# roclark/torchsr

Hardware: AMD Instinct MI355X
Metric: 96x96 HR crops/sec (SRGAN GAN train step) (higher is better)
Workload: dtype f32; 1 GPU; SRGAN full GAN step (Generator + Discriminator + VGG19 perceptual loss), 96x96 HR crops, batch 16 per GPU, fp32; per_gpu_batch=16, global_batch=16, crop=96, parallelism=dp1, hip_graph=True, vgg19_weights=seeded-random, plan_cus=256

## Files before the change

include/srx.h:

```cpp
#ifndef SRX_H
#define SRX_H

#include <stddef.h>
#include <stdint.h>

#ifdef __cplusplus
extern "C" {
#endif

#define SRX_VERSION 100

enum {
  SRX_OK = 0,
  SRX_E_BADARG = 1,
  SRX_E_UNSUPPORTED = 2,
  SRX_E_HIP = 3,
  SRX_E_WORKSPACE = 4
};

enum { SRX_ACT_NONE = 0, SRX_ACT_RELU = 1, SRX_ACT_LRELU = 2, SRX_ACT_PRELU = 3 };

int srx_version(void);
int srx_last_error(char* buf, size_t n);
int srx_build_info(char* buf, size_t n);
// ... 35 lines not shown
} srx_conv2d_t;

size_t srx_conv2d_packed_fwd_floats(const srx_conv2d_t* d);
size_t srx_conv2d_packed_bwd_floats(const srx_conv2d_t* d);
size_t srx_conv2d_fwd_ws_floats(const srx_conv2d_t* d);
size_t srx_conv2d_bwd_data_ws_floats(const srx_conv2d_t* d);
size_t srx_conv2d_bwd_weight_ws_floats(const srx_conv2d_t* d);
int srx_conv2d_stat_rows(const srx_conv2d_t* d);

int srx_conv2d_plan(const srx_conv2d_t* d, int which, int* out);

int srx_conv2d_force_plan(int bm, int bn, int split, int ks);
int srx_conv2d_force_s2(int mode, int bm, int bn);
int srx_wgrad_force(int lin, int nsplit);
int srx_wgrad_force_kernels(int dma, int rows, int reduce);
int srx_thin_force_rows(int rows);
int srx_linear_force(int form, int splits);

int srx_thin_plan(const srx_conv2d_t* d, int which, int* out);

int srx_linear_plan(int B, int K, int J, int which, int* out);

int srx_wgrad_plan(const srx_conv2d_t* d, int nprob, int per_out, int* out);

int srx_conv2d_pack(const srx_conv2d_t* d, const float* w_oihw, float* wpk_fwd, float* wpk_bwd, void* stream);

size_t srx_pack_table_bytes(int n_layers);
int srx_pack_table_build(const srx_conv2d_t* descs, int n, const float* const* w_oihw, float* const* wpk_fwd,
                         float* const* wpk_bwd, void* host_table, int* n_records, long long* max_elems);
int srx_pack_table_run(const void* dev_table, int n_records, long long max_elems, void* stream);
// ... 277 lines not shown
```

torchsr_amd/_lib.py:

```python
import ctypes as C
import os
import subprocess
import sys

_HERE = os.path.dirname(os.path.abspath(__file__))
CSRC = os.path.join(_HERE, 'csrc')
LIB_PATH = os.environ.get('SRX_LIB') or os.path.join(CSRC, 'libsrx_hip.so')
SOURCES = ['api.cpp', 'gconv.hip', 'wgrad.hip', 'convpack.hip', 'c64.hip', 'thin9.hip', 'rdb.hip', 'thin.hip', 'rowtile.hip', 'augment.hip', 'degrade.hip', 'norm.hip', 'eltwise.hip', 'linear.hip', 'loss.hip', 'head.hip', 'wino.hip', 'optim.hip', 'dihedral.hip', 'resample.hip', 'usm.hip', 'pool.hip', 'colorfix.hip', 'compact.hip', 'specnorm.hip']
HEADERS = ['srx_common.h', 'conv_host.h', os.path.join('..', '..', 'include', 'srx.h')]

ACT_NONE, ACT_RELU, ACT_LRELU, ACT_PRELU = 0, 1, 2, 3


class Conv2dDesc(C.Structure):
    _fields_ = [
        ('N', C.c_int32), ('H', C.c_int32), ('W', C.c_int32),
        ('Cin', C.c_int32), ('Cin_s', C.c_int32), ('Cout', C.c_int32), ('Cout_s', C.c_int32),
        ('KH', C.c_int32), ('KW', C.c_int32), ('stride', C.c_int32), ('pad', C.c_int32),
        ('shuffle', C.c_int32), ('act', C.c_int32), ('slope', C.c_float), ('up', C.c_int32),
        ('precision', C.c_int32),
    ]


class DgradEpilogue(C.Structure):
# ... 120 lines not shown
    'srx_plane_moments': (_I, [_P, _L, _I, _I, _P, _Z, _P, _P]),
    'srx_color_fix_adain_apply': (_I, [_P, _P, _L, _I, _I, _P, _P, _P]),
    'srx_conv2d_packed_fwd_floats': (_Z, [_D]),
    'srx_conv2d_packed_bwd_floats': (_Z, [_D]),
    'srx_conv2d_fwd_ws_floats': (_Z, [_D]),
    'srx_conv2d_bwd_data_ws_floats': (_Z, [_D]),
    'srx_conv2d_bwd_weight_ws_floats': (_Z, [_D]),
    'srx_conv2d_stat_rows': (_I, [_D]),
    'srx_conv2d_plan': (_I, [_D, _I, C.POINTER(C.c_int)]),
    'srx_conv2d_force_plan': (_I, [_I, _I, _I, _I]),
    'srx_thin_plan': (_I, [_D, _I, C.POINTER(C.c_int)]),
    'srx_thin_force_rows': (_I, [_I]),
    'srx_conv2d_force_s2': (_I, [_I, _I, _I]),
    'srx_wgrad_force': (_I, [_I, _I]),
    'srx_wgrad_force_kernels': (_I, [_I, _I, _I]),
    'srx_wgrad_plan': (_I, [_D, _I, _I, C.POINTER(C.c_int)]),
    'srx_linear_force': (_I, [_I, _I]),
    'srx_linear_plan': (_I, [_I, _I, _I, _I, C.POINTER(C.c_int)]),
    'srx_pack_table_bytes': (_Z, [_I]),
    'srx_pack_table_build': (_I, [_P, _I, _P, _P, _P, _P, C.POINTER(C.c_int), C.POINTER(C.c_longlong)]),
    'srx_pack_table_add_wino': (_I, [_P, C.POINTER(C.c_int), C.POINTER(C.c_longlong), _D, _P, _P, _I]),
    'srx_pack_table_run': (_I, [_P, _I, C.c_longlong, _P]),
    'srx_conv2d_pack': (_I, [_D, _P, _P, _P, _P]),
    'srx_conv2d_fwd': (_I, [_D, _P, _P, _P, _P, _P, _P, _Z, _P]),
    'srx_conv3x3_c64_bf16_packed_bytes': (_Z, [_I]),
    'srx_conv3x3_c64_bf16_pack': (_I, [_P, _P, _P, _I, _I, _P, _P]),
    'srx_conv3x3_c64_bf16_fwd': (_I, [_I, _I, _I, _I, _I, _P, _P, _F, _P, _P, _I, _P]),
    'srx_conv3x3_c64_bf16_plan': (_I, [_I, _I, _I, _I, C.POINTER(C.c_int)]),
    'srx_f32_to_bf16': (_I, [_P, _P, _L, _P]),
    'srx_bf16_to_f32': (_I, [_P, _P, _L, _P]),
# ... 200 lines not shown
```

torchsr_amd/csrc/api.cpp:

```cpp
#include "srx_common.h"
#include <cstdarg>
#include <cstdio>
#include <atomic>
#include <cstdlib>
#include <cstring>
#include <mutex>
#include <vector>

static thread_local char g_err[512] = "";

void srx_set_error(const char* fmt, ...) {
  va_list ap;
  va_start(ap, fmt);
  vsnprintf(g_err, sizeof(g_err), fmt, ap);
  va_end(ap);
}

extern "C" int srx_version(void) { return SRX_VERSION; }

#ifndef SRX_SOURCES_SHA256
#define SRX_SOURCES_SHA256 "unknown"
#endif
static const char g_build_info[] = "srx-build-sources-sha256:" SRX_SOURCES_SHA256;
extern "C" int srx_build_info(char* buf, size_t n) {
// ... 3 lines not shown
  return SRX_OK;
}

static SrxDevSwitches read_switches() {
  SrxDevSwitches s{};
  auto flag = [](const char* n) { const char* e = getenv(n); return e != nullptr && e[0] != 0 && !(e[0] == '0' && e[1] == 0); };
  auto num = [](const char* n) { const char* e = getenv(n); return e ? atoi(e) : 0; };
  s.no_rt36 = flag("SRX_NO_RT36");
  s.no_wgrad_rows = flag("SRX_NO_WGRAD_ROWS");
  s.no_bn_bwd_fuse = flag("SRX_NO_BN_BWD_FUSE");
  s.no_bn_fwd_fuse = flag("SRX_NO_BN_FWD_FUSE");
  s.no_first3 = flag("SRX_NO_FIRST3");
  s.no_c64 = flag("SRX_NO_C64");
  s.no_wgrad_dma = flag("SRX_NO_WGRAD_DMA");
  s.no_wgrad_lin = flag("SRX_NO_WGRAD_LIN");
  s.wgrad_nsplit = num("SRX_WGRAD_NSPLIT");
  s.wgrad_rows_nsplit = num("SRX_WGRAD_ROWS_NSPLIT");
  s.first3_wgs_per_cu = num("SRX_FIRST3_WGS_PER_CU");
  s.thin_fwd_rows = num("SRX_THIN_FWD_ROWS");
  s.reserved_cus = num("SRX_RESERVED_CUS");
  s.c64_ablate = num("SRX_C64_ABLATE");
  s.rdb_ablate = num("SRX_RDB_ABLATE");
  s.no_wino = flag("SRX_NO_WINO");
  s.old_wgrad_reduce = flag("SRX_OLD_WGRAD_REDUCE");
  s.wino_no_tail = flag("SRX_WINO_NO_TAIL");
  s.wino_zsplit = num("SRX_WINO_ZSPLIT");
  s.wino_bn = num("SRX_WINO_BN");
  s.s2_mode = num("SRX_S2_MODE");
  if (s.rdb_ablate != 0 || s.c64_ablate != 0) {
    const char* ok = getenv("SRX_ALLOW_GARBAGE_RESULTS");
// ... 142 lines not shown
```

torchsr_amd/csrc/conv_host.h:

```cpp
#pragma once
#include "srx_common.h"
#include <atomic>

constexpr int BK = 32;

struct Geo {
  int Ho, Wo, Ck, K, Kp, Cnp, cps;
};

struct BwdClass {
  int ph, pw, nth, ntw, dminh, dminw, Hm, Wm, K, Kp;
  size_t woff;
};

int check_desc(const srx_conv2d_t* d);
bool small_enough(const srx_conv2d_t* d);
int pad_rows(int c);
Geo fwd_geo(const srx_conv2d_t* d);
int bwd_ck(const srx_conv2d_t* d);
int bwd_classes(const srx_conv2d_t* d, BwdClass* cls, size_t& total_floats);
srx_conv2d_t upsampled_desc(const srx_conv2d_t* d);
size_t upsampled_floats(const srx_conv2d_t* d);

struct ConvForce {
  std::atomic<int> plan[4];
  std::atomic<int> s2[3];
  std::atomic<int> wg[2];
  std::atomic<int> wg_rows;
  std::atomic<int> wk[3];
};
ConvForce& conv_force();
```

torchsr_amd/csrc/gconv.hip:

```cpp
#include "conv_host.h"
#include <cstdio>
#include <cstdlib>
#include <algorithm>
#include <mutex>
#include <type_traits>
#include <utility>
#include <vector>

namespace {

struct GArgs {
  const float* in; const float* w; const float* bias; float* out; float* part;
  int N, Hi, Wi, Ci;
  int Hm, Wm, M, HmWm;
  float inv_HmWm, inv_Wm;
  int in_stride, nth, ntw, dh0, dw0, Ck, K, Kp;
  int Cn, Cs;
  int Ho, Wo, Co;
  int out_stride, oh_off, ow_off;
  int out_shuffle, in_shuffle;
  int up;
  int act; float slope;
  int linear_out;
  int mtiles;
// ... 1067 lines not shown
  srx_conv2d_t h = *d;
  h.up = 0; h.H = 2 * d->H; h.W = 2 * d->W;
  return h;
}
size_t upsampled_floats(const srx_conv2d_t* d) { return (size_t)d->N * 2 * d->H * 2 * d->W * d->Cin_s; }

ConvForce& conv_force() {
  static ConvForce* f = [] {
    ConvForce* s = new ConvForce;
    const SrxDevSwitches& e = srx_dev();
    for (int i = 0; i < 4; ++i) s->plan[i].store(e.force_plan ? e.plan[i] : 0);
    s->s2[0].store((e.s2_mode & 1) ? 1 : 0); s->s2[1].store(0); s->s2[2].store(0);
    s->wg[0].store(e.no_wgrad_lin ? 0 : -1); s->wg[1].store(e.wgrad_nsplit > 0 && e.wgrad_nsplit <= 64 ? e.wgrad_nsplit : 0);
    s->wg_rows.store(e.wgrad_rows_nsplit > 0 && e.wgrad_rows_nsplit <= 64 ? e.wgrad_rows_nsplit : 0);
    s->wk[0].store(e.no_wgrad_dma ? 0 : -1); s->wk[1].store(e.no_wgrad_rows ? 0 : -1); s->wk[2].store(e.old_wgrad_reduce ? 0 : -1);
    return s;
  }();
  return *f;
}

namespace {

struct Plan { int BM, BN, mtiles, ntiles, tiles, full, tail, split, kc_per_split, ks; float cost; bool refused; };

enum Family { F_GCONV, F_BIG, F_MULTI, F_S2F, NFAM };
constexpr unsigned char K1 = 1, K2 = 2, K4 = 4, K12 = K1 | K2;
struct Tile {
  int BM, BN, WM, WN, XR;
  float eff;
  unsigned char ks[NFAM][4];
// ... 489 lines not shown

extern "C" int srx_conv2d_force_s2(int mode, int bm, int bn) {
  SRX_REQUIRE(((mode == 0 || mode == 1) && bm == 0 && bn == 0) ||
              (mode == 2 && ((bm == 0 && bn == 0) || tile_sides_known(F_S2F, bm, bn))),
              "conv2d_force_s2: (0, 0, 0), (1, 0, 0) or (2, BM 64 / 128 / 144, BN 64 / 128) -- (2, 0, 0): the model's fused tile");
  ConvForce& f = conv_force();
  f.s2[0].store(0);
  f.s2[1].store(bm); f.s2[2].store(bn); f.s2[0].store(mode);
  return SRX_OK;
}

extern "C" int srx_wgrad_force(int lin, int nsplit) {
  SRX_REQUIRE(lin >= -1 && lin <= 1 && nsplit >= 0 && nsplit <= 64, "wgrad_force: LIN -1 / 0 / 1, 0..64 row splits");
  ConvForce& f = conv_force();
  f.wg[0].store(lin); f.wg[1].store(nsplit); f.wg_rows.store(nsplit);
  return SRX_OK;
}

extern "C" int srx_wgrad_force_kernels(int dma, int rows, int reduce) {
  SRX_REQUIRE(dma >= -1 && dma <= 1 && rows >= -1 && rows <= 1 && reduce >= -1 && reduce <= 1,
              "wgrad_force_kernels: DMA staging, image-row kernel, row-wise reduction: each -1 / 0 / 1");
  ConvForce& f = conv_force();
  f.wk[0].store(dma); f.wk[1].store(rows); f.wk[2].store(reduce);
  return SRX_OK;
}

static int conv_fwd_impl(const srx_conv2d_t* d, const float* x, const float* wpk, const float* bias, const float* residual,
                         float out_scale, float* y, float* bn_partials, float* ws, size_t ws_floats, void* stream) {
  if (int rc = check_desc(d)) return rc;
  SRX_REQUIRE(x && wpk && y, "conv2d_fwd: null pointer");
// ... 360 lines not shown
```

torchsr_amd/csrc/srx_common.h:

```cpp
#pragma once
#include <hip/hip_runtime.h>
#include <hip/hip_ext.h>
#include <stdint.h>
#include <stddef.h>
#include "../../include/srx.h"

typedef float f32x4 __attribute__((ext_vector_type(4)));
typedef float f32x16 __attribute__((ext_vector_type(16)));

void srx_set_error(const char* fmt, ...);

#define SRX_FAIL(code, ...)      \
  do {                           \
    srx_set_error(__VA_ARGS__);  \
    return (code);               \
  } while (0)

#define SRX_REQUIRE(cond, ...) \
  do {                         \
    if (!(cond)) SRX_FAIL(SRX_E_BADARG, __VA_ARGS__); \
  } while (0)

#define SRX_CHECK_LAUNCH(name)                                                        \
  do {                                                                                \
    hipError_t e__ = hipGetLastError();                                               \
    if (e__ != hipSuccess) SRX_FAIL(SRX_E_HIP, "%s: %s", name, hipGetErrorString(e__)); \
  } while (0)

struct SrxDevSwitches {
  bool no_rt36, no_wgrad_rows, no_bn_bwd_fuse, no_bn_fwd_fuse, no_first3, no_c64, force_plan, no_wgrad_dma, no_wgrad_lin, no_wino, old_wgrad_reduce, wino_no_tail;
  int wgrad_nsplit, wgrad_rows_nsplit, first3_wgs_per_cu, thin_fwd_rows, reserved_cus, c64_ablate, rdb_ablate, wino_zsplit, wino_bn;
  int s2_mode;
  int plan[4];
};
const SrxDevSwitches& srx_dev();
extern "C" int srx_plan_cus(void);

bool srx_prof_on();
bool srx_prof_aux();
bool srx_prof_take(const char* name, double flops, hipEvent_t* e0, hipEvent_t* e1);
#define SRX_LAUNCH_PROF(name, flops, kernel, grid, block, lds, st, ...)                              \
  do {                                                                                               \
    hipEvent_t e0__ = nullptr, e1__ = nullptr;                                                       \
    if (srx_prof_on() && srx_prof_take(name, flops, &e0__, &e1__))                                   \
      hipExtLaunchKernelGGL(kernel, grid, block, (std::uint32_t)(lds), st, e0__, e1__, 0, __VA_ARGS__); \
// ... 91 lines not shown
```

torchsr_amd/csrc/wgrad.hip:

```cpp
#include "conv_host.h"
#include <cstdio>

namespace {

struct WArgs {
  const float* in; const float* dy; float* slab;
  int N, Hi, Wi, Ci, Hm, Wm, M, HmWm;
  float inv_HmWm, inv_Wm;
  int in_stride, nth, ntw, dh0, dw0, Ck, K, Kw;
  int Cd, Cdv, dy_shuffle, Cnw;
  int rows_per_split, ktiles;
  unsigned in_bytes, dy_bytes;
  int s_c, s_rm, dX0, dX1, dX2, dD0, dD1;
  float* bslab;
  int nsplit, nprob;
};

constexpr int WG_MAXP = 72;
struct WMulti {
  WArgs a;
  const float* x[WG_MAXP];
  const float* dy[WG_MAXP];
};
struct WReduce {
// ... 178 lines not shown
  }
  if (want_bias) {
    f32x4* red = reinterpret_cast<f32x4*>(&sD[0][0]);
    red[r0 * 16 + q] = bsum;
    __syncthreads();
    if (tid < 16) {
      f32x4 t = red[tid];
#pragma unroll
      for (int r = 1; r < 16; ++r) t += red[r * 16 + tid];
      *reinterpret_cast<f32x4*>(a.bslab + slab_id * a.Cnw + n0 + 4 * tid) = t;
    }
  }
}

constexpr int WG_MASKW = 768;
template <bool WIDE, bool LIN = false>
__global__ __launch_bounds__(256) void wgrad_dma_kernel(const WMulti mp) {
  static_assert(!LIN || WIDE, "LIN is a form of WIDE");
  const WArgs& a = mp.a;
  typedef unsigned u32x4 __attribute__((ext_vector_type(4)));
  int wi;
  {
    const int W = (int)gridDim.x, b = (int)blockIdx.x, xcd = b & 7, slot = b >> 3, q = W >> 3, r = W & 7;
    wi = (xcd < r ? xcd * (q + 1) : r * (q + 1) + (xcd - r) * q) + slot;
  }
  const int tiles_ = a.ktiles * (a.Cnw / 64);
  const int tile_id = wi % tiles_, rest_ = wi / tiles_;
  const int prob = srx_uniform(rest_ % a.nprob), zsplit = srx_uniform(rest_ / a.nprob);
  constexpr int NSLOT = 3, CHUNK = 32 * 64;
  __shared__ __attribute__((aligned(16))) float sD[NSLOT][CHUNK];
  __shared__ __attribute__((aligned(16))) float sX[NSLOT][CHUNK];
  const int tid = threadIdx.x, lane = tid & 63, wave = srx_uniform(tid >> 6);
  const int ntile = srx_uniform(tile_id / a.ktiles), kt = srx_uniform(tile_id - ntile * a.ktiles);
  const int k0 = kt * 64, n0 = ntile * 64;
  constexpr int NP = WIDE ? 1 : 2;
  const int q = WIDE ? (tid & 7) : (tid & 15), r0 = WIDE ? (tid >> 3) : (tid >> 4);
  auto make_rsrc = [](const void* p, unsigned bytes) {
    const unsigned long long v = (unsigned long long)p;
    u32x4 r;
    r[0] = (unsigned)srx_uniform((int)(unsigned)v);
    r[1] = (unsigned)srx_uniform((int)((unsigned)(v >> 32) & 0xffffu));
    r[2] = bytes;
    r[3] = 0x00020000u;
    return r;
  };
  const u32x4 rx_ = make_rsrc(mp.x[prob], a.in_bytes), rd_ = make_rsrc(mp.dy[prob], a.dy_bytes);

  const int k = k0 + 4 * q;
  const bool kvalid = k < a.K, kvalid1 = WIDE && k + 32 < a.K;
  int dh = 0, dw = 0, kc = 0;
  if (kvalid) {
    const int tap = k / a.Ck;
    kc = k - tap * a.Ck;
    const int th = tap / a.ntw, tw = tap - th * a.ntw;
    dh = a.dh0 + th;
    dw = a.dw0 + tw;
  }
  const int col = n0 + 4 * q;
  const bool cvalid = col < a.Cdv, cvalid1 = WIDE && col + 32 < a.Cdv;
  int sh_i = 0, sh_j = 0, sh_c = col;
  if (a.dy_shuffle) {
    const int ij = col / a.dy_shuffle;
    sh_c = col - ij * a.dy_shuffle;
    sh_i = ij >> 1;
    sh_j = ij & 1;
  }
  const int mbeg = zsplit * a.rows_per_split;
  const int mend = min(a.M, mbeg + a.rows_per_split);

  __shared__ unsigned okmask[LIN ? WG_MASKW : 1];
  if constexpr (LIN) {
    const int nrows = (((mend - mbeg + 31) / 32 + 3) * 32 + 63) & ~63;
    for (int base = wave * 64; base < nrows; base += 256) {
      const int m = mbeg + base + lane;
      int n, rem, mh, mw;
      srx_divmod(m, a.HmWm, a.inv_HmWm, n, rem);
      srx_divmod(rem, a.Wm, a.inv_Wm, mh, mw);
      const bool ok = m < mend && ((unsigned)(mh + dh) < (unsigned)a.Hi) && ((unsigned)(mw + dw) < (unsigned)a.Wi);
      const unsigned long long bits = __ballot(ok);
      if (lane == 0) { okmask[base >> 5] = (unsigned)bits; okmask[(base >> 5) + 1] = (unsigned)(bits >> 32); }
// ... 8 lines not shown
    int n, rem, mh, mw;
    srx_divmod(m, a.HmWm, a.inv_HmWm, n, rem);
    srx_divmod(rem, a.Wm, a.inv_Wm, mh, mw);
    rm[p] = m; rmh[p] = mh; rmw[p] = mw;
    rox[p] = (unsigned)(((n * a.Hi + mh * a.in_stride + dh) * a.Wi + mw * a.in_stride + dw) * a.Ci + kc);
    rod[p] = (unsigned)(a.dy_shuffle ? ((n * 2 * a.Hm + 2 * mh + sh_i) * (2 * a.Wm) + 2 * mw + sh_j) * a.Cd + sh_c
                                     : m * a.Cd + col);
  }
  const unsigned ldsX = (unsigned)(size_t)&sX[0][0], ldsD = (unsigned)(size_t)&sD[0][0];
  auto dma = [&](const u32x4& rs, unsigned voff, unsigned dst) {
    unsigned keep;
    asm volatile("s_mov_b32 %0, m0\n\ts_mov_b32 m0, %2\n\ts_nop 0\n\tbuffer_load_dwordx4 %1, %3, 0 offen lds\n\ts_mov_b32 m0, %0"
                 : "=&s"(keep) : "v"(voff), "s"(dst), "s"(rs) : "memory");
  };
  constexpr unsigned OORL = 0xfffff000u;
  unsigned lin_x = 0, lin_d = 0, lin_w = 0;
  int lin_c = 0;
  if constexpr (LIN) {
    lin_x = 4u * (unsigned)((mbeg + r0 + dh * a.Wi + dw) * a.Ci + kc);
    lin_d = 4u * (unsigned)((mbeg + r0) * a.Cd + col);
    lin_w = okmask[0];
  }
  const unsigned lin_sx = 128u * (unsigned)a.Ci, lin_sd = 128u * (unsigned)a.Cd;
  auto request = [&](int slot) {
    if constexpr (LIN) {
      const bool okx = (lin_w >> r0) & 1u;
      const bool okd = rm[0] < mend;
      const unsigned vx = okx ? lin_x : OORL, vd = okd ? lin_d : OORL;
      const unsigned dst = (unsigned)srx_uniform((int)((unsigned)(slot * CHUNK * 4) + (unsigned)(wave * 1024)));
      dma(rx_, vx, ldsX + dst);
      dma(rd_, vd, ldsD + dst);
      dma(rx_, vx + 128u, ldsX + dst + 4096u);
      dma(rd_, vd + 128u, ldsD + dst + 4096u);
      rm[0] += 32; lin_x += lin_sx; lin_d += lin_sd;
      lin_c += 1;
      lin_w = okmask[lin_c];
      return;
    }
#pragma unroll
    for (int p = 0; p < NP; ++p) {
      const bool valid = rm[p] < mend;
      const int ih = rmh[p] * a.in_stride + dh, iw = rmw[p] * a.in_stride + dw;
      const bool okx = valid && kvalid && ((unsigned)ih < (unsigned)a.Hi) && ((unsigned)iw < (unsigned)a.Wi);
      const unsigned dst = (unsigned)srx_uniform((int)((unsigned)(slot * CHUNK * 4) + (unsigned)(p * 4096 + wave * 1024)));
      dma(rx_, okx ? 4u * rox[p] : 0xffffffffu, ldsX + dst);
      dma(rd_, (valid && cvalid) ? 4u * rod[p] : 0xffffffffu, ldsD + dst);
      if constexpr (WIDE) {
        dma(rx_, (okx && kvalid1) ? 4u * rox[p] + 128u : 0xffffffffu, ldsX + dst + 4096u);
        dma(rd_, (valid && cvalid1) ? 4u * rod[p] + 128u : 0xffffffffu, ldsD + dst + 4096u);
      }
      rm[p] += 32; rmw[p] += a.s_c; rmh[p] += a.s_rm; rox[p] += (unsigned)a.dX0; rod[p] += (unsigned)a.dD0;
      const bool wc = rmw[p] >= a.Wm;
      rmw[p] -= wc ? a.Wm : 0; rmh[p] += wc ? 1 : 0;
      rox[p] += wc ? (unsigned)a.dX1 : 0u; rod[p] += wc ? (unsigned)a.dD1 : 0u;
      const bool wr = rmh[p] >= a.Hm;
      rmh[p] -= wr ? a.Hm : 0;
      rox[p] += wr ? (unsigned)a.dX2 : 0u;
    }
  };
  const bool want_bias = a.bslab != nullptr && kt == 0;
  f32x4 bsum = {0.f, 0.f, 0.f, 0.f}, bsum1 = {0.f, 0.f, 0.f, 0.f};
  f32x16 acc;
#pragma unroll
  for (int r = 0; r < 16; ++r) acc[r] = 0.f;
  const int h = lane >> 5, l31 = lane & 31;
  const int wn = wave >> 1, wk = wave & 1;
  constexpr int SSTEP = WIDE ? 64 : 128, HSTEP = WIDE ? 32 : 64, WSTEP = WIDE ? 1024 : 32;
  auto compute = [&](int slot) {
    const float* cD = &sD[0][0] + slot * CHUNK + h * HSTEP + wn * WSTEP + l31;
    const float* cX = &sX[0][0] + slot * CHUNK + h * HSTEP + wk * WSTEP + l31;
    if (want_bias) {
      if constexpr (WIDE) {
        const float* bd = &sD[0][0] + slot * CHUNK + r0 * 32 + q * 4;
        bsum += *reinterpret_cast<const f32x4*>(bd);
        bsum1 += *reinterpret_cast<const f32x4*>(bd + 1024);
      } else {
        const float* bd = &sD[0][0] + slot * CHUNK + r0 * 64 + q * 4;
        bsum += *reinterpret_cast<const f32x4*>(bd) + *reinterpret_cast<const f32x4*>(bd + 16 * 64);
      }
    }
    float dv[16], xv[16];
#pragma unroll
    for (int s = 0; s < 16; ++s) { dv[s] = cD[s * SSTEP]; xv[s] = cX[s * SSTEP]; }
#pragma unroll
    for (int s = 0; s < 16; ++s) acc = __builtin_amdgcn_mfma_f32_32x32x2f32(dv[s], xv[s], acc, 0, 0, 0);
    __builtin_amdgcn_sched_group_barrier(0x100, 4, 0);
#pragma unroll
    for (int i = 0; i < 8; ++i) {
      __builtin_amdgcn_sched_group_barrier(0x008, 2, 0);
      if (i < 6) __builtin_amdgcn_sched_group_barrier(0x100, 2, 0);
    }
  };
  const int nchunks = (mend - mbeg + 31) / 32;
  request(0);
  request(1);
  asm volatile("s_waitcnt vmcnt(4)" ::: "memory");
  asm volatile("s_waitcnt lgkmcnt(0)\n\ts_barrier" ::: "memory");
  int slot = 0;
  for (int c = 0; c < nchunks; ++c) {
    int s2 = slot + 2; s2 = s2 >= NSLOT ? s2 - NSLOT : s2;
    request(s2);
    compute(slot);
    asm volatile("s_waitcnt vmcnt(4)" ::: "memory");
    asm volatile("s_waitcnt lgkmcnt(0)\n\ts_barrier" ::: "memory");
    slot = slot + 1 == NSLOT ? 0 : slot + 1;
  }
  asm volatile("s_waitcnt vmcnt(0)" ::: "memory");
  const size_t slab_id = (size_t)prob * a.nsplit + zsplit;
  float* slab = a.slab + slab_id * a.Cnw * a.Kw;
#pragma unroll
  for (int r = 0; r < 16; ++r) {
    const int row = n0 + wn * 32 + (r & 3) + 8 * (r >> 2) + 4 * h;
    slab[(size_t)row * a.Kw + k0 + wk * 32 + l31] = acc[r];
  }
  if (want_bias) {
    __syncthreads();
    f32x4* red = reinterpret_cast<f32x4*>(&sD[0][0]);
    constexpr int NR = WIDE ? 32 : 16;
    if constexpr (WIDE) { red[r0 * 16 + q] = bsum; red[r0 * 16 + 8 + q] = bsum1; }
    else red[r0 * 16 + q] = bsum;
    __syncthreads();
    if (tid < 16) {
      f32x4 t = red[tid];
#pragma unroll
      for (int r = 1; r < NR; ++r) t += red[r * 16 + tid];
      *reinterpret_cast<f32x4*>(a.bslab + slab_id * a.Cnw + n0 + 4 * tid) = t;
    }
  }
}

template <int WPX>
__global__ __launch_bounds__(256) void wgrad_rows_bf16_kernel(const WMulti mp) {
  const WArgs& a = mp.a;
  typedef __bf16 bf16x4 __attribute__((ext_vector_type(4)));
  typedef __bf16 bf16x8 __attribute__((ext_vector_type(8)));
  typedef short s16x4 __attribute__((ext_vector_type(4)));
  typedef short s16x8 __attribute__((ext_vector_type(8)));
  typedef s16x4 __attribute__((address_space(3))) * lds_s16x4;
  constexpr int XPS = 64, XROW = (WPX + 2) * XPS;
  constexpr int DPS = 192, DROW = WPX * DPS;
// ... 250 lines not shown
    if (e < nE) {
      const int ci = e / T, tap = e - ci * T;
      const float v = rsum[tap * Ck + ci];
      orow[e] = accumulate ? oldv[i] + v : v;
    }
  }
  for (int e = tid + 256 * PRE; e < nE; e += 256) {
    const int ci = e / T, tap = e - ci * T;
    const float v = rsum[tap * Ck + ci];
    orow[e] = accumulate ? orow[e] + v : v;
  }
}

}

static int wgrad_nsplit(int M, int64_t tiles, int nprob, int Cnw, int Kw, int precision) {
  const int cus = srx_plan_cus();
  const int max_by_rows = (int)srx_cdiv(M, 128);
  int nsplit = 1;
  float best_cost = 1e30f;
  for (int ns = 1; ns <= 64 && ns <= max_by_rows; ++ns) {
    const int rps = (int)srx_roundup(srx_cdiv(M, ns), 32);
    if ((int)srx_cdiv(M, rps) != ns) continue;
    float cost;
    if (precision == 0) {
      const int w = (int)srx_cdiv(tiles * nprob * ns, cus), f = w / 3, r = w - 3 * f;
      cost = (rps / 32 + 3.5f) * (f * 1.696f + (r == 1 ? 0.633f : r == 2 ? 1.177f : 0.f)) + (float)nprob * ns * Cnw * Kw * 8.0f / 50.0e6f;
    } else {
      const int L = (int)srx_cdiv(tiles * nprob * ns, cus);
      const float hide = L >= 4 ? 0.65f : (L == 3 ? 0.7f : (L == 2 ? 0.8f : 1.0f));
      cost = 1.07f * L * (rps / 32 + 6) * hide + (float)nprob * ns * Cnw * Kw * 8.0f / 3.0e6f;
    }
    if (cost < best_cost) { best_cost = cost; nsplit = ns; }
  }
  if (const int v = conv_force().wg[1].load(std::memory_order_relaxed); v > 0) {
    const int rps = (int)srx_roundup(srx_cdiv(M, v), 32);
    if (v > max_by_rows || (int)srx_cdiv(M, rps) != v) {
      srx_set_error("conv2d_bwd_weight: forced %d row splits refused: %d rows split into whole 32-row chunks of at least 128 rows "
                    "give %d splits", v, M, v > max_by_rows ? max_by_rows : (int)srx_cdiv(M, rps));
      return -1;
    }
    nsplit = v;
  }
  const int rps = (int)srx_roundup(srx_cdiv(M, nsplit), 32);
  return (int)srx_cdiv(M, rps);
}

static bool wgrad_rows_ok(const srx_conv2d_t* d) {
  if (conv_force().wk[1].load(std::memory_order_relaxed) == 0 || !d->precision || d->KH != 3 || d->KW != 3 || d->stride != 1 || d->pad != 1 || d->shuffle || d->up == 2) return false;
  return d->Cout == 64 && srx_roundup(d->Cin, 4) % 32 == 0 && (d->W == 32 || d->W == 16);
}
static int wgrad_rows_nsplit(const srx_conv2d_t* d, int nprob) {
  const int cus = srx_plan_cus();
  const int groups = (int)srx_roundup(d->Cin, 4) / 32, rows = d->N * d->H;
  int best = 1;
  float best_cost = 1e30f;
  for (int ns = 1; ns <= 32 && ns <= rows; ++ns) {
    const int rps = (int)srx_cdiv(rows, ns);
// ... 10 lines not shown
    }
    best = v;
  }
  const int rps = (int)srx_cdiv(rows, best);
  return (int)srx_cdiv(rows, rps);
}

enum { WK_F32 = 0, WK_DMA = 1, WK_DMA_WIDE = 2, WK_DMA_LIN = 3, WK_BF16 = 4, WK_ROWS32 = 5, WK_ROWS16 = 6, WK_THIN = 7 };
struct WgradPlan {
  int kernel;
  int nsplit;
  int rows_per_split;
  int reduce;
  int workgroups;
  int Cnw, Kw;
};
static int wgrad_plan(const srx_conv2d_t* d, int nprob, WgradPlan& p) {
  const Geo g = fwd_geo(d);
  const ConvForce& f = conv_force();
  p.Cnw = (int)srx_roundup(d->Cout, 64);
  p.Kw = (int)srx_roundup(g.K, 64);
  const int M = d->N * g.Ho * g.Wo;
  const int64_t tiles = (int64_t)(p.Kw / 64) * (p.Cnw / 64);
  if (wgrad_rows_ok(d)) {
    p.nsplit = wgrad_rows_nsplit(d, nprob);
    if (p.nsplit < 0) return SRX_E_UNSUPPORTED;
    p.kernel = d->W == 32 ? WK_ROWS32 : WK_ROWS16;
    p.rows_per_split = (int)srx_cdiv(d->N * d->H, p.nsplit) * d->W;
    p.workgroups = (g.Ck / 32) * nprob * p.nsplit;
  } else {
    p.nsplit = wgrad_nsplit(M, tiles, nprob, p.Cnw, p.Kw, d->precision);
    if (p.nsplit < 0) return SRX_E_UNSUPPORTED;
    p.rows_per_split = (int)srx_roundup(srx_cdiv(M, p.nsplit), 32);
    p.workgroups = (int)(tiles * nprob * p.nsplit);
    if (d->precision) {
      p.kernel = WK_BF16;
    } else if (f.wk[0].load(std::memory_order_relaxed) == 0) {
      p.kernel = WK_F32;
    } else {
      p.kernel = WK_DMA;
      const int Cdv = bwd_ck(d);
      if (g.Ck % 64 == 0 && Cdv % 64 == 0 && (!g.cps || g.cps % 64 == 0)) {
        const size_t in_bytes = (size_t)d->N * d->H * d->W * d->Cin_s * sizeof(float);
        const size_t dy_bytes = (size_t)M * (d->shuffle ? 4 : 1) * d->Cout_s * sizeof(float);
        const bool lin = f.wg[0].load(std::memory_order_relaxed) != 0 && d->stride == 1 && d->H == g.Ho && d->W == g.Wo && !g.cps &&
                         g.K % 64 == 0 && p.rows_per_split / 32 + 3 <= WG_MASKW && in_bytes < 0xfff00000ull && dy_bytes < 0xfff00000ull;
        p.kernel = lin ? WK_DMA_LIN : WK_DMA_WIDE;
      }
    }
  }
  p.reduce = (f.wk[2].load(std::memory_order_relaxed) == 0 || (size_t)g.K * sizeof(float) > 48 * 1024) ? 0 : 1;
  return SRX_OK;
}

extern "C" int srx_wgrad_plan(const srx_conv2d_t* d, int nprob, int per_out, int* out) {
  if (int rc = check_desc(d)) return rc;
  SRX_REQUIRE(out && nprob >= 1 && nprob <= WG_MAXP && per_out >= 1 && nprob % per_out == 0,
// ... 125 lines not shown
  const double wfl = 2.0 * a.M * d->Cout * a.K * nprob;
  char nm[112];
  if (rows_kernel) {
    if (srx_prof_on()) snprintf(nm, sizeof(nm), "wgrad_rows_bf16_kernel<%d> MxNxK=%dx%dx%d x%d", d->W, a.M, d->Cout, a.K, nprob);
    if (plan.kernel == WK_ROWS32) SRX_LAUNCH_PROF(nm, wfl, wgrad_rows_bf16_kernel<32>, grid, dim3(256), 0, st, mp);
    else SRX_LAUNCH_PROF(nm, wfl, wgrad_rows_bf16_kernel<16>, grid, dim3(256), 0, st, mp);
    SRX_CHECK_LAUNCH("wgrad_rows_bf16_kernel");
  } else {
    const int form = plan.kernel;
    if (srx_prof_on()) {
      if (form == WK_F32 || form == WK_BF16) snprintf(nm, sizeof(nm), "wgrad_kernel<%d> MxNxK=%dx%dx%d x%d", form == WK_BF16 ? 1 : 0, a.M, d->Cout, a.K, nprob);
      else snprintf(nm, sizeof(nm), "wgrad_dma_kernel<%d, %d> MxNxK=%dx%dx%d x%d", form >= WK_DMA_WIDE ? 1 : 0, form == WK_DMA_LIN ? 1 : 0, a.M, d->Cout, a.K, nprob);
    }
    if (form == WK_BF16) SRX_LAUNCH_PROF(nm, wfl, wgrad_kernel<1>, grid, dim3(256), 0, st, mp);
    else if (form == WK_F32) SRX_LAUNCH_PROF(nm, wfl, wgrad_kernel<0>, grid, dim3(256), 0, st, mp);
    else if (form == WK_DMA_LIN) SRX_LAUNCH_PROF(nm, wfl, (wgrad_dma_kernel<true, true>), grid, dim3(256), 0, st, mp);
    else if (form == WK_DMA_WIDE) SRX_LAUNCH_PROF(nm, wfl, wgrad_dma_kernel<true>, grid, dim3(256), 0, st, mp);
    else SRX_LAUNCH_PROF(nm, wfl, wgrad_dma_kernel<false>, grid, dim3(256), 0, st, mp);
    SRX_CHECK_LAUNCH("wgrad_kernel");
  }
  if (plan.reduce == 0) {
    const int64_t n = (int64_t)d->Cout * g.K;
    SRX_LAUNCH_PROF_AUX("wgrad_reduce_kernel", wgrad_reduce_kernel, dim3((unsigned)srx_cdiv(n, 256), (unsigned)nout), dim3(256), 0, st, ws,
                    nsplit * per_out, a.Cnw, a.Kw, g.K, g.Ck, d->Cout, d->Cin, d->KH, d->KW, g.cps, outs, accumulate,
                    a.bslab);
  } else {
    SRX_LAUNCH_PROF_AUX("wgrad_reduce_rows_kernel", wgrad_reduce_rows_kernel, dim3((unsigned)d->Cout, (unsigned)nout), dim3(256),
                    (size_t)g.K * sizeof(float), st, ws, nsplit * per_out, a.Cnw, a.Kw, g.K, g.Ck, d->Cout, d->Cin, d->KH, d->KW, g.cps,
                    outs, accumulate, a.bslab);
  }
// ... 37 lines not shown
```

Measured before the change: 2444 crops/s.

## Add 128x64 tall tile variant to fp32 DMA wgrad kernel with cost-model selection

Adds a TALL template form of the fp32 DMA weight-gradient kernel. Each workgroup computes 128 output channels by 64 K columns, with two MFMA accumulators sharing the same input operand loads. This halves X-tile reloads and workgroup count per output tile. A cost model extension picks the tall tile for eligible 3x3 layers when its estimated cost beats the standard tile by a margin. The trade is more LDS and registers per workgroup, which lowers occupancy, and the selection relies on new empirical constants.

```diff
diff --git a/include/srx.h b/include/srx.h
--- a/include/srx.h
+++ b/include/srx.h
@@ -73,6 +73,7 @@
 int srx_conv2d_force_s2(int mode, int bm, int bn);
 int srx_wgrad_force(int lin, int nsplit);
 int srx_wgrad_force_kernels(int dma, int rows, int reduce);
+int srx_wgrad_force_tile(int tall);
 int srx_thin_force_rows(int rows);
 int srx_linear_force(int form, int splits);
 
diff --git a/torchsr_amd/_lib.py b/torchsr_amd/_lib.py
--- a/torchsr_amd/_lib.py
+++ b/torchsr_amd/_lib.py
@@ -158,6 +158,7 @@
     'srx_conv2d_force_s2': (_I, [_I, _I, _I]),
     'srx_wgrad_force': (_I, [_I, _I]),
     'srx_wgrad_force_kernels': (_I, [_I, _I, _I]),
+    'srx_wgrad_force_tile': (_I, [_I]),
     'srx_wgrad_plan': (_I, [_D, _I, _I, C.POINTER(C.c_int)]),
     'srx_linear_force': (_I, [_I, _I]),
     'srx_linear_plan': (_I, [_I, _I, _I, _I, C.POINTER(C.c_int)]),
diff --git a/torchsr_amd/csrc/api.cpp b/torchsr_amd/csrc/api.cpp
--- a/torchsr_amd/csrc/api.cpp
+++ b/torchsr_amd/csrc/api.cpp
@@ -41,6 +41,7 @@
   s.no_c64 = flag("SRX_NO_C64");
   s.no_wgrad_dma = flag("SRX_NO_WGRAD_DMA");
   s.no_wgrad_lin = flag("SRX_NO_WGRAD_LIN");
+  s.no_wgrad_tall = flag("SRX_NO_WGRAD_TALL");
   s.wgrad_nsplit = num("SRX_WGRAD_NSPLIT");
   s.wgrad_rows_nsplit = num("SRX_WGRAD_ROWS_NSPLIT");
   s.first3_wgs_per_cu = num("SRX_FIRST3_WGS_PER_CU");
diff --git a/torchsr_amd/csrc/conv_host.h b/torchsr_amd/csrc/conv_host.h
--- a/torchsr_amd/csrc/conv_host.h
+++ b/torchsr_amd/csrc/conv_host.h
@@ -28,5 +28,6 @@
   std::atomic<int> wg[2];
   std::atomic<int> wg_rows;
   std::atomic<int> wk[3];
+  std::atomic<int> wg_tile;
 };
 ConvForce& conv_force();
diff --git a/torchsr_amd/csrc/gconv.hip b/torchsr_amd/csrc/gconv.hip
--- a/torchsr_amd/csrc/gconv.hip
+++ b/torchsr_amd/csrc/gconv.hip
@@ -1105,6 +1105,7 @@
     s->wg[0].store(e.no_wgrad_lin ? 0 : -1); s->wg[1].store(e.wgrad_nsplit > 0 && e.wgrad_nsplit <= 64 ? e.wgrad_nsplit : 0);
     s->wg_rows.store(e.wgrad_rows_nsplit > 0 && e.wgrad_rows_nsplit <= 64 ? e.wgrad_rows_nsplit : 0);
     s->wk[0].store(e.no_wgrad_dma ? 0 : -1); s->wk[1].store(e.no_wgrad_rows ? 0 : -1); s->wk[2].store(e.old_wgrad_reduce ? 0 : -1);
+    s->wg_tile.store(e.no_wgrad_tall ? 0 : -1);
     return s;
   }();
   return *f;
@@ -1624,6 +1625,12 @@
   SRX_REQUIRE(lin >= -1 && lin <= 1 && nsplit >= 0 && nsplit <= 64, "wgrad_force: LIN -1 / 0 / 1, 0..64 row splits");
   ConvForce& f = conv_force();
   f.wg[0].store(lin); f.wg[1].store(nsplit); f.wg_rows.store(nsplit);
+  return SRX_OK;
+}
+
+extern "C" int srx_wgrad_force_tile(int tall) {
+  SRX_REQUIRE(tall >= -1 && tall <= 1, "wgrad_force_tile: the 128 x 64 tile -1 (the cost model) / 0 (never) / 1 (wherever eligible)");
+  conv_force().wg_tile.store(tall);
   return SRX_OK;
 }
 
diff --git a/torchsr_amd/csrc/srx_common.h b/torchsr_amd/csrc/srx_common.h
--- a/torchsr_amd/csrc/srx_common.h
+++ b/torchsr_amd/csrc/srx_common.h
@@ -28,7 +28,7 @@
   } while (0)
 
 struct SrxDevSwitches {
-  bool no_rt36, no_wgrad_rows, no_bn_bwd_fuse, no_bn_fwd_fuse, no_first3, no_c64, force_plan, no_wgrad_dma, no_wgrad_lin, no_wino, old_wgrad_reduce, wino_no_tail;
+  bool no_rt36, no_wgrad_rows, no_bn_bwd_fuse, no_bn_fwd_fuse, no_first3, no_c64, force_plan, no_wgrad_dma, no_wgrad_lin, no_wgrad_tall, no_wino, old_wgrad_reduce, wino_no_tail;
   int wgrad_nsplit, wgrad_rows_nsplit, first3_wgs_per_cu, thin_fwd_rows, reserved_cus, c64_ablate, rdb_ablate, wino_zsplit, wino_bn;
   int s2_mode;
   int plan[4];
diff --git a/torchsr_amd/csrc/wgrad.hip b/torchsr_amd/csrc/wgrad.hip
--- a/torchsr_amd/csrc/wgrad.hip
+++ b/torchsr_amd/csrc/wgrad.hip
@@ -216,9 +216,11 @@
 }
 
 constexpr int WG_MASKW = 768;
-template <bool WIDE, bool LIN = false>
+template <bool WIDE, bool LIN = false, bool TALL = false>
 __global__ __launch_bounds__(256) void wgrad_dma_kernel(const WMulti mp) {
   static_assert(!LIN || WIDE, "LIN is a form of WIDE");
+  static_assert(!TALL || WIDE, "TALL is a form of WIDE");
+  static_assert(WG_MASKW % 2 == 0, "the bit table is filled two words at a time");
   const WArgs& a = mp.a;
   typedef unsigned u32x4 __attribute__((ext_vector_type(4)));
   int wi;
@@ -226,15 +228,16 @@
     const int W = (int)gridDim.x, b = (int)blockIdx.x, xcd = b & 7, slot = b >> 3, q = W >> 3, r = W & 7;
     wi = (xcd < r ? xcd * (q + 1) : r * (q + 1) + (xcd - r) * q) + slot;
   }
-  const int tiles_ = a.ktiles * (a.Cnw / 64);
+  constexpr int TN = TALL ? 128 : 64;
+  const int tiles_ = a.ktiles * (a.Cnw / TN);
   const int tile_id = wi % tiles_, rest_ = wi / tiles_;
   const int prob = srx_uniform(rest_ % a.nprob), zsplit = srx_uniform(rest_ / a.nprob);
-  constexpr int NSLOT = 3, CHUNK = 32 * 64;
-  __shared__ __attribute__((aligned(16))) float sD[NSLOT][CHUNK];
+  constexpr int NSLOT = 3, CHUNK = 32 * 64, DCHUNK = 32 * TN;
+  __shared__ __attribute__((aligned(16))) float sD[NSLOT][DCHUNK];
   __shared__ __attribute__((aligned(16))) float sX[NSLOT][CHUNK];
   const int tid = threadIdx.x, lane = tid & 63, wave = srx_uniform(tid >> 6);
   const int ntile = srx_uniform(tile_id / a.ktiles), kt = srx_uniform(tile_id - ntile * a.ktiles);
-  const int k0 = kt * 64, n0 = ntile * 64;
+  const int k0 = kt * 64, n0 = ntile * TN;
   constexpr int NP = WIDE ? 1 : 2;
   const int q = WIDE ? (tid & 7) : (tid & 15), r0 = WIDE ? (tid >> 3) : (tid >> 4);
   auto make_rsrc = [](const void* p, unsigned bytes) {
@@ -260,12 +263,18 @@
   }
   const int col = n0 + 4 * q;
   const bool cvalid = col < a.Cdv, cvalid1 = WIDE && col + 32 < a.Cdv;
+  const bool cvalid2 = TALL && col + 64 < a.Cdv, cvalid3 = TALL && col + 96 < a.Cdv;
   int sh_i = 0, sh_j = 0, sh_c = col;
+  unsigned dd2 = 64u;
   if (a.dy_shuffle) {
     const int ij = col / a.dy_shuffle;
     sh_c = col - ij * a.dy_shuffle;
     sh_i = ij >> 1;
     sh_j = ij & 1;
+    if constexpr (TALL) {
+      const int ij2 = (col + 64) / a.dy_shuffle, c2 = col + 64 - ij2 * a.dy_shuffle;
+      dd2 = (unsigned)((((ij2 >> 1) - sh_i) * (2 * a.Wm) + (ij2 & 1) - sh_j) * a.Cd + c2 - sh_c);
+    }
   }
   const int mbeg = zsplit * a.rows_per_split;
   const int mend = min(a.M, mbeg + a.rows_per_split);
@@ -304,6 +313,7 @@
                  : "=&s"(keep) : "v"(voff), "s"(dst), "s"(rs) : "memory");
   };
   constexpr unsigned OORL = 0xfffff000u;
+  static_assert(OORL >= 0xfff00000u && OORL + 128u + 256u > OORL, "OORL must stay out of range under every added offset");
   unsigned lin_x = 0, lin_d = 0, lin_w = 0;
   int lin_c = 0;
   if constexpr (LIN) {
@@ -318,10 +328,15 @@
       const bool okd = rm[0] < mend;
       const unsigned vx = okx ? lin_x : OORL, vd = okd ? lin_d : OORL;
       const unsigned dst = (unsigned)srx_uniform((int)((unsigned)(slot * CHUNK * 4) + (unsigned)(wave * 1024)));
+      const unsigned dstd = (unsigned)srx_uniform((int)((unsigned)(slot * DCHUNK * 4) + (unsigned)(wave * 1024)));
       dma(rx_, vx, ldsX + dst);
-      dma(rd_, vd, ldsD + dst);
+      dma(rd_, vd, ldsD + dstd);
       dma(rx_, vx + 128u, ldsX + dst + 4096u);
-      dma(rd_, vd + 128u, ldsD + dst + 4096u);
+      dma(rd_, vd + 128u, ldsD + dstd + 4096u);
+      if constexpr (TALL) {
+        dma(rd_, vd + 256u, ldsD + dstd + 8192u);
+        dma(rd_, vd + 384u, ldsD + dstd + 12288u);
+      }
       rm[0] += 32; lin_x += lin_sx; lin_d += lin_sd;
       lin_c += 1;
       lin_w = okmask[lin_c];
@@ -333,11 +348,16 @@
       const int ih = rmh[p] * a.in_stride + dh, iw = rmw[p] * a.in_stride + dw;
       const bool okx = valid && kvalid && ((unsigned)ih < (unsigned)a.Hi) && ((unsigned)iw < (unsigned)a.Wi);
       const unsigned dst = (unsigned)srx_uniform((int)((unsigned)(slot * CHUNK * 4) + (unsigned)(p * 4096 + wave * 1024)));
+      const unsigned dstd = (unsigned)srx_uniform((int)((unsigned)(slot * DCHUNK * 4) + (unsigned)(p * 4096 + wave * 1024)));
       dma(rx_, okx ? 4u * rox[p] : 0xffffffffu, ldsX + dst);
-      dma(rd_, (valid && cvalid) ? 4u * rod[p] : 0xffffffffu, ldsD + dst);
+      dma(rd_, (valid && cvalid) ? 4u * rod[p] : 0xffffffffu, ldsD + dstd);
       if constexpr (WIDE) {
         dma(rx_, (okx && kvalid1) ? 4u * rox[p] + 128u : 0xffffffffu, ldsX + dst + 4096u);
-        dma(rd_, (valid && cvalid1) ? 4u * rod[p] + 128u : 0xffffffffu, ldsD + dst + 4096u);
+        dma(rd_, (valid && cvalid1) ? 4u * rod[p] + 128u : 0xffffffffu, ldsD + dstd + 4096u);
+      }
+      if constexpr (TALL) {
+        dma(rd_, (valid && cvalid2) ? 4u * (rod[p] + dd2) : 0xffffffffu, ldsD + dstd + 8192u);
+        dma(rd_, (valid && cvalid3) ? 4u * (rod[p] + dd2) + 128u : 0xffffffffu, ldsD + dstd + 12288u);
       }
       rm[p] += 32; rmw[p] += a.s_c; rmh[p] += a.s_rm; rox[p] += (unsigned)a.dX0; rod[p] += (unsigned)a.dD0;
       const bool wc = rmw[p] >= a.Wm;
@@ -349,27 +369,48 @@
     }
   };
   const bool want_bias = a.bslab != nullptr && kt == 0;
-  f32x4 bsum = {0.f, 0.f, 0.f, 0.f}, bsum1 = {0.f, 0.f, 0.f, 0.f};
-  f32x16 acc;
-#pragma unroll
-  for (int r = 0; r < 16; ++r) acc[r] = 0.f;
+  f32x4 bsum = {0.f, 0.f, 0.f, 0.f}, bsum1 = {0.f, 0.f, 0.f, 0.f}, bsum2 = {0.f, 0.f, 0.f, 0.f}, bsum3 = {0.f, 0.f, 0.f, 0.f};
+  f32x16 acc, acc2;
+#pragma unroll
+  for (int r = 0; r < 16; ++r) { acc[r] = 0.f; acc2[r] = 0.f; }
   const int h = lane >> 5, l31 = lane & 31;
   const int wn = wave >> 1, wk = wave & 1;
   constexpr int SSTEP = WIDE ? 64 : 128, HSTEP = WIDE ? 32 : 64, WSTEP = WIDE ? 1024 : 32;
   auto compute = [&](int slot) {
-    const float* cD = &sD[0][0] + slot * CHUNK + h * HSTEP + wn * WSTEP + l31;
+    const float* cD = &sD[0][0] + slot * DCHUNK + h * HSTEP + wn * WSTEP + l31;
     const float* cX = &sX[0][0] + slot * CHUNK + h * HSTEP + wk * WSTEP + l31;
     if (want_bias) {
       if constexpr (WIDE) {
-        const float* bd = &sD[0][0] + slot * CHUNK + r0 * 32 + q * 4;
+        const float* bd = &sD[0][0] + slot * DCHUNK + r0 * 32 + q * 4;
         bsum += *reinterpret_cast<const f32x4*>(bd);
         bsum1 += *reinterpret_cast<const f32x4*>(bd + 1024);
+        if constexpr (TALL) {
+          bsum2 += *reinterpret_cast<const f32x4*>(bd + 2048);
+          bsum3 += *reinterpret_cast<const f32x4*>(bd + 3072);
+        }
       } else {
         const float* bd = &sD[0][0] + slot * CHUNK + r0 * 64 + q * 4;
         bsum += *reinterpret_cast<const f32x4*>(bd) + *reinterpret_cast<const f32x4*>(bd + 16 * 64);
       }
     }
     float dv[16], xv[16];
+    if constexpr (TALL) {
+      float ev[16];
+#pragma unroll
+      for (int s = 0; s < 16; ++s) { dv[s] = cD[s * SSTEP]; ev[s] = cD[s * SSTEP + 2048]; xv[s] = cX[s * SSTEP]; }
+#pragma unroll
+      for (int s = 0; s < 16; ++s) {
+        acc = __builtin_amdgcn_mfma_f32_32x32x2f32(dv[s], xv[s], acc, 0, 0, 0);
+        acc2 = __builtin_amdgcn_mfma_f32_32x32x2f32(ev[s], xv[s], acc2, 0, 0, 0);
+      }
+      __builtin_amdgcn_sched_group_barrier(0x100, 6, 0);
+#pragma unroll
+      for (int i = 0; i < 8; ++i) {
+        __builtin_amdgcn_sched_group_barrier(0x008, 4, 0);
+        if (i < 6) __builtin_amdgcn_sched_group_barrier(0x100, 3, 0);
+      }
+      return;
+    }
 #pragma unroll
     for (int s = 0; s < 16; ++s) { dv[s] = cD[s * SSTEP]; xv[s] = cX[s * SSTEP]; }
 #pragma unroll
@@ -381,17 +422,21 @@
       if (i < 6) __builtin_amdgcn_sched_group_barrier(0x100, 2, 0);
     }
   };
+  auto wait_newest = [] {
+    if constexpr (TALL) asm volatile("s_waitcnt vmcnt(6)" ::: "memory");
+    else asm volatile("s_waitcnt vmcnt(4)" ::: "memory");
+  };
   const int nchunks = (mend - mbeg + 31) / 32;
   request(0);
   request(1);
-  asm volatile("s_waitcnt vmcnt(4)" ::: "memory");
+  wait_newest();
   asm volatile("s_waitcnt lgkmcnt(0)\n\ts_barrier" ::: "memory");
   int slot = 0;
   for (int c = 0; c < nchunks; ++c) {
     int s2 = slot + 2; s2 = s2 >= NSLOT ? s2 - NSLOT : s2;
     request(s2);
     compute(slot);
-    asm volatile("s_waitcnt vmcnt(4)" ::: "memory");
+    wait_newest();
     asm volatile("s_waitcnt lgkmcnt(0)\n\ts_barrier" ::: "memory");
     slot = slot + 1 == NSLOT ? 0 : slot + 1;
   }
@@ -402,18 +447,21 @@
   for (int r = 0; r < 16; ++r) {
     const int row = n0 + wn * 32 + (r & 3) + 8 * (r >> 2) + 4 * h;
     slab[(size_t)row * a.Kw + k0 + wk * 32 + l31] = acc[r];
+    if constexpr (TALL) slab[(size_t)(row + 64) * a.Kw + k0 + wk * 32 + l31] = acc2[r];
   }
   if (want_bias) {
     __syncthreads();
     f32x4* red = reinterpret_cast<f32x4*>(&sD[0][0]);
     constexpr int NR = WIDE ? 32 : 16;
-    if constexpr (WIDE) { red[r0 * 16 + q] = bsum; red[r0 * 16 + 8 + q] = bsum1; }
+    constexpr int NQ = TN / 4;
+    if constexpr (TALL) { red[r0 * 32 + q] = bsum; red[r0 * 32 + 8 + q] = bsum1; red[r0 * 32 + 16 + q] = bsum2; red[r0 * 32 + 24 + q] = bsum3; }
+    else if constexpr (WIDE) { red[r0 * 16 + q] = bsum; red[r0 * 16 + 8 + q] = bsum1; }
     else red[r0 * 16 + q] = bsum;
     __syncthreads();
-    if (tid < 16) {
+    if (tid < NQ) {
       f32x4 t = red[tid];
 #pragma unroll
-      for (int r = 1; r < NR; ++r) t += red[r * 16 + tid];
+      for (int r = 1; r < NR; ++r) t += red[r * NQ + tid];
       *reinterpret_cast<f32x4*>(a.bslab + slab_id * a.Cnw + n0 + 4 * tid) = t;
     }
   }
@@ -694,8 +742,19 @@
 
 }
 
-static int wgrad_nsplit(int M, int64_t tiles, int nprob, int Cnw, int Kw, int precision) {
+constexpr float WG_TALL_ROUND2 = 2.097f, WG_TALL_ROUND1 = 1.165f, WG_TALL_FILL = 3.75f, WG_TALL_MARGIN = 6.4f;
+static int wgrad_nsplit(int M, int64_t tiles, int nprob, int Cnw, int Kw, int precision, bool tall, float* cost_out) {
   const int cus = srx_plan_cus();
+  auto fp32_cost = [&](int ns, int rps) {
+    const float slabs = (float)nprob * ns * Cnw * Kw * 8.0f / 50.0e6f;
+    const int w = (int)srx_cdiv(tiles * nprob * ns, cus);
+    if (tall) {
+      const int f = w / 2, r = w - 2 * f;
+      return (rps / 32 + WG_TALL_FILL) * (f * WG_TALL_ROUND2 + r * WG_TALL_ROUND1) + slabs;
+    }
+    const int f = w / 3, r = w - 3 * f;
+    return (rps / 32 + 3.5f) * (f * 1.696f + (r == 1 ? 0.633f : r == 2 ? 1.177f : 0.f)) + slabs;
+  };
   const int max_by_rows = (int)srx_cdiv(M, 128);
   int nsplit = 1;
   float best_cost = 1e30f;
@@ -704,8 +763,7 @@
     if ((int)srx_cdiv(M, rps) != ns) continue;
     float cost;
     if (precision == 0) {
-      const int w = (int)srx_cdiv(tiles * nprob * ns, cus), f = w / 3, r = w - 3 * f;
-      cost = (rps / 32 + 3.5f) * (f * 1.696f + (r == 1 ? 0.633f : r == 2 ? 1.177f : 0.f)) + (float)nprob * ns * Cnw * Kw * 8.0f / 50.0e6f;
+      cost = fp32_cost(ns, rps);
     } else {
       const int L = (int)srx_cdiv(tiles * nprob * ns, cus);
       const float hide = L >= 4 ? 0.65f : (L == 3 ? 0.7f : (L == 2 ? 0.8f : 1.0f));
@@ -721,7 +779,9 @@
       return -1;
     }
     nsplit = v;
-  }
+    best_cost = precision == 0 ? fp32_cost(v, rps) : 0.f;
+  }
+  if (cost_out) *cost_out = best_cost;
   const int rps = (int)srx_roundup(srx_cdiv(M, nsplit), 32);
   return (int)srx_cdiv(M, rps);
 }
@@ -762,6 +822,7 @@
   int reduce;
   int workgroups;
   int Cnw, Kw;
+  bool tall;
 };
 static int wgrad_plan(const srx_conv2d_t* d, int nprob, WgradPlan& p) {
   const Geo g = fwd_geo(d);
@@ -770,6 +831,7 @@
   p.Kw = (int)srx_roundup(g.K, 64);
   const int M = d->N * g.Ho * g.Wo;
   const int64_t tiles = (int64_t)(p.Kw / 64) * (p.Cnw / 64);
+  p.tall = false;
   if (wgrad_rows_ok(d)) {
     p.nsplit = wgrad_rows_nsplit(d, nprob);
     if (p.nsplit < 0) return SRX_E_UNSUPPORTED;
@@ -777,18 +839,27 @@
     p.rows_per_split = (int)srx_cdiv(d->N * d->H, p.nsplit) * d->W;
     p.workgroups = (g.Ck / 32) * nprob * p.nsplit;
   } else {
-    p.nsplit = wgrad_nsplit(M, tiles, nprob, p.Cnw, p.Kw, d->precision);
+    const int Cdv = bwd_ck(d);
+    const bool dma = !d->precision && f.wk[0].load(std::memory_order_relaxed) != 0;
+    const bool wide = dma && g.Ck % 64 == 0 && Cdv % 64 == 0 && (!g.cps || g.cps % 64 == 0);
+    float cost = 0.f;
+    p.nsplit = wgrad_nsplit(M, tiles, nprob, p.Cnw, p.Kw, d->precision, false, &cost);
     if (p.nsplit < 0) return SRX_E_UNSUPPORTED;
+    if (const int ft = f.wg_tile.load(std::memory_order_relaxed); ft != 0 && wide && p.Cnw % 128 == 0 && Cdv % 128 == 0) {
+      float tcost = 0.f;
+      const int tns = wgrad_nsplit(M, tiles / 2, nprob, p.Cnw, p.Kw, 0, true, &tcost);
+      if (tns < 0) return SRX_E_UNSUPPORTED;
+      if (ft == 1 || (d->KH == 3 && d->KW == 3 && tcost + WG_TALL_MARGIN < cost)) { p.tall = true; p.nsplit = tns; }
+    }
     p.rows_per_split = (int)srx_roundup(srx_cdiv(M, p.nsplit), 32);
-    p.workgroups = (int)(tiles * nprob * p.nsplit);
+    p.workgroups = (int)((p.tall ? tiles / 2 : tiles) * nprob * p.nsplit);
     if (d->precision) {
       p.kernel = WK_BF16;
     } else if (f.wk[0].load(std::memory_order_relaxed) == 0) {
       p.kernel = WK_F32;
     } else {
       p.kernel = WK_DMA;
-      const int Cdv = bwd_ck(d);
-      if (g.Ck % 64 == 0 && Cdv % 64 == 0 && (!g.cps || g.cps % 64 == 0)) {
+      if (wide) {
         const size_t in_bytes = (size_t)d->N * d->H * d->W * d->Cin_s * sizeof(float);
         const size_t dy_bytes = (size_t)M * (d->shuffle ? 4 : 1) * d->Cout_s * sizeof(float);
         const bool lin = f.wg[0].load(std::memory_order_relaxed) != 0 && d->stride == 1 && d->H == g.Ho && d->W == g.Wo && !g.cps &&
@@ -944,6 +1015,8 @@
     }
     if (form == WK_BF16) SRX_LAUNCH_PROF(nm, wfl, wgrad_kernel<1>, grid, dim3(256), 0, st, mp);
     else if (form == WK_F32) SRX_LAUNCH_PROF(nm, wfl, wgrad_kernel<0>, grid, dim3(256), 0, st, mp);
+    else if (form == WK_DMA_LIN && plan.tall) SRX_LAUNCH_PROF(nm, wfl, (wgrad_dma_kernel<true, true, true>), grid, dim3(256), 0, st, mp);
+    else if (form == WK_DMA_WIDE && plan.tall) SRX_LAUNCH_PROF(nm, wfl, (wgrad_dma_kernel<true, false, true>), grid, dim3(256), 0, st, mp);
     else if (form == WK_DMA_LIN) SRX_LAUNCH_PROF(nm, wfl, (wgrad_dma_kernel<true, true>), grid, dim3(256), 0, st, mp);
     else if (form == WK_DMA_WIDE) SRX_LAUNCH_PROF(nm, wfl, wgrad_dma_kernel<true>, grid, dim3(256), 0, st, mp);
     else SRX_LAUNCH_PROF(nm, wfl, wgrad_dma_kernel<false>, grid, dim3(256), 0, st, mp);
```

New measurement: 2436 crops/s. About the same (-0.3%).
